# ElBaldo1/FastOptSolver

Measured on AMD Instinct MI355X. Metric: fista_iterations_per_second, higher is better.
Workload: dtype f32

## Files before the change

### fastoptsolver_amd/_core.py

```python
import ctypes as C
import collections
import math

import numpy as np
import torch

from . import _lib


def require_gpu():
    if not torch.cuda.is_available():
        raise _lib.FosError("fastoptsolver_amd needs a ROCm GPU (torch.cuda.is_available() is False); "
                            "there is no CPU fallback by design")


def stream_ptr():
    return C.c_void_p(torch.cuda.current_stream().cuda_stream)


def ptr(t):
    return C.c_void_p(t.data_ptr()) if t is not None else C.c_void_p(0)


def is_tensor(x):
# ... 416 lines not shown

    def plan(self):
        arr = (C.c_int32 * 8)()
        _lib.check(self.lib.fos_problem_plan(self.h, arr), "fos_problem_plan")
        keys = ("path", "threads", "chunks", "rows", "workgroups", "slabs", "nontemporal", "cus")
        plan = dict(zip(keys, list(arr)))
        flags = plan["nontemporal"]
        plan["nontemporal"] = flags & 1
        plan["resident"] = (flags >> 1) & 1
        plan["tall"] = (flags >> 2) & 1
        plan["colblock"] = (flags >> 3) & 1
        plan["cluster"] = (flags >> 4) & 1
        plan["interleave"] = (flags >> 5) & 1
        plan["fused_mfma"] = (flags >> 6) & 1
        plan["chip_resident"] = (flags >> 7) & 1
        return plan

    def replan(self, no_resident=False, no_tall=False, no_wide=False, no_colblock=False, cluster=None, interleave=None,
               fused_mfma=False, chip_resident=None):
        flags = ((_lib.PLAN_NO_RESIDENT if no_resident else 0) | (_lib.PLAN_NO_TALL if no_tall else 0) |
                 (_lib.PLAN_NO_WIDE if no_wide else 0) | (_lib.PLAN_NO_COLBLOCK if no_colblock else 0) |
                 (0 if cluster is None else (_lib.PLAN_CLUSTER if cluster else _lib.PLAN_NO_CLUSTER)) |
                 (0 if interleave is None else (_lib.PLAN_INTERLEAVE if interleave else _lib.PLAN_NO_INTERLEAVE)) |
                 (_lib.PLAN_FUSED_MFMA if fused_mfma else 0) |
                 (0 if chip_resident is None else (_lib.PLAN_CHIP_RESIDENT if chip_resident else _lib.PLAN_NO_CHIP_RESIDENT)))
        with self.ctx():
            _lib.check(self.lib.fos_problem_replan(self.h, flags), "fos_problem_replan")

    def set_comm(self, comm):
        _lib.check(self.lib.fos_problem_set_comm(self.h, comm.h if comm is not None else None), "fos_problem_set_comm")
        self.comm = comm

    def set_comm_cols(self, comm):
        with self.ctx():
            _lib.check(self.lib.fos_problem_set_comm_cols(self.h, comm.h), "fos_problem_set_comm_cols")
        self.comm = comm
        self.col_sharded = True

    def tune(self, threads, chunks, rows, workgroups=0):
        _lib.check(self.lib.fos_problem_tune(self.h, threads, chunks, rows, workgroups), "fos_problem_tune")
# ... 399 lines not shown
```

### fastoptsolver_amd/_lib.py

```python
import ctypes as C
import os

HERE = os.path.dirname(os.path.abspath(__file__))
LIB_PATH = os.path.join(HERE, "libfos_hip.so")

FOS_F32, FOS_BF16 = 0, 1
MODE_FISTA, MODE_DELTA, MODE_ISTA = 0, 1, 2
PROX_L1, PROX_ENET = 0, 1
LOSS_SQUARED, LOSS_LOGISTIC = 0, 1
LOSS_MULTINOMIAL = 2
STOP_NONE, STOP_STEP, STOP_RATIO, STOP_GRAD, STOP_LS_STALL = 0, 1, 2, 3, 4
ERR_UNSUPPORTED = -4
PLAN_NO_RESIDENT, PLAN_NO_TALL, PLAN_NO_WIDE, PLAN_NO_COLBLOCK, PLAN_CLUSTER, PLAN_INTERLEAVE, PLAN_NO_INTERLEAVE, PLAN_NO_CLUSTER, PLAN_FUSED_MFMA, PLAN_CHIP_RESIDENT, PLAN_NO_CHIP_RESIDENT = 1, 2, 4, 8, 16, 32, 64, 128, 256, 512, 1024


class FistaParams(C.Structure):
    _fields_ = [("tau", C.c_double), ("alpha1", C.c_double), ("alpha2", C.c_double), ("delta", C.c_double),
                ("restart_threshold", C.c_double), ("tol_step", C.c_double), ("tol_ratio", C.c_double),
                ("tol_grad", C.c_double), ("mode", C.c_int32), ("prox_kind", C.c_int32), ("adaptive_restart", C.c_int32),
                ("group", C.c_int32)]


class LineSearchState(C.Structure):
    _fields_ = [(k, C.c_double) for k in ("f0", "d0", "dtest", "width", "width1", "lo", "flo", "dlo", "hi", "fhi", "dhi",
                                           "smin", "smax")] + [(k, C.c_int32) for k in ("stage1", "brackt", "status", "reserved")]


class LbfgsResult(C.Structure):
# ... 161 lines not shown
```

### fastoptsolver_amd/csrc/fos_fista.hip

```cpp
#include "fos_internal.hpp"
#include "fused_step.hpp"
#include "chip_resident.hpp"
#include <cassert>

using namespace fosapi;

template <int NQ>
static int launch_fused(const fos::FusedArgs& a, int G, size_t lds, hipStream_t st) {
  auto kern = fos::fista_fused_kernel<NQ>;
  static std::atomic<uint64_t> done{0};
  int dev = 0;
  HIP_TRY(hipGetDevice(&dev));
  const uint64_t bit = 1ull << (dev & 63);
  if (!(done.load(std::memory_order_acquire) & bit)) {
    HIP_TRY(hipFuncSetAttribute(reinterpret_cast<const void*>(kern), hipFuncAttributeMaxDynamicSharedMemorySize, (int)lds));
    done.fetch_or(bit, std::memory_order_release);
  }
  hipLaunchKernelGGL(kern, dim3(G), dim3(fos::FZ_THREADS), lds, st, a);
  LAUNCH_CHECK();
  return FOS_OK;
}

template <int NC, bool CTRL>
static int launch_chip(const fos::ChipArgs& a, int G, size_t lds, hipStream_t st) {
// ... 402 lines not shown
  hipLaunchKernelGGL(fos::history_fold_kernel, dim3(iters), dim3(64), 0, p->stream, rr2_slots, nwg, part_slots, f->nupd,
                     hist);
  LAUNCH_CHECK();
  rc = finish_plain(f, part_slots + (iters - 1) * psz, iters >= 2 ? part_slots + (iters - 2) * psz : nullptr, f->nupd,
                    p->pass.rr_part, nwg);
  restart_plain(f);
  return rc;
}

int fos_fista_run(fos_fista* f, int iters) {
  if (!f || iters < 0) return fail(FOS_ERR_ARG, "fos_fista_run: bad argument");
  if (int rc_ = need_squared(f->p, "fos_fista_run")) return rc_;
  if (int rc_ = need_separable(f, "fos_fista_run")) return rc_;
  fos_problem* p = f->p;
  if (iters == 0) return FOS_OK;
  if (p->pass.resident) return run_resident(f, iters, nullptr, nullptr);
  {
    const bool chip_region = p->dtype == FOS_F32 && p->m >= 512 && iters >= 8 &&
                             (p->n <= 8 ? p->m <= 131072 : (p->n <= 16 && p->m <= 32768));
    if ((p->chip_mode == 1 || (p->chip_mode == 0 && chip_region)) && !p->comm && !f->precise && !f->prm.tau_from_state &&
        f->prm.tol_grad == 0.0) {
      const int rcc = fos_fista_run_chip(f, iters);
      if (rcc != FOS_ERR_UNSUPPORTED && rcc != FOS_ERR_STATE) return rcc;
    }
  }
  if (f->prm.tol_grad > 0.0 && !p->comm) {
    for (int it = 0; it < iters; ++it) {
      int rc;
      if ((rc = fos_fista_grad(f))) return rc;
      if ((rc = launch_grad_norm_stop(f))) return rc;
// ... 717 lines not shown
                       (int)p->cand.n_pad, f->x_cur, f->x_prev, f->scal, f->prm, t, eta, nv, p->cand.xp, p->ws.part, t_from_state);
  hipLaunchKernelGGL(fos::fold_partials_kernel, dim3(1), dim3(fos::FOLD_THREADS), 0, p->stream, p->ws.part, grid, fos::BT_W, p->cand.bt_out);
  LAUNCH_CHECK();
  if (p->col_sharded) {
    int rc = reduce_across(p, p->cand.bt_out, fos::BT_W, true);
    if (rc) return rc;
  }
  return launch_residual_batch(p, 0, p->cand.bt_out + 64, stopped);
}

static int run_device_driven(fos_fista* f, int iters, bool backtracking, double eta, double armijo_c, double grad_eps,
                             int32_t* ls_iters, double* tau_hist, double* x_hist, double* hist, double* rr_seen) {
  fos_problem* p = f->p;
  int rc = flush_pending(f);
  if (rc) return rc;
  if (backtracking) {
    if ((rc = ensure_batch_workspace(p))) return rc;
    if (!f->tau_on_device) {
      hipLaunchKernelGGL(fos::set_state_tau_kernel, dim3(1), dim3(1), 0, p->stream, f->scal, f->prm.tau);
      LAUNCH_CHECK();
      f->tau_on_device = true;
    }
  }
  hand_to_device(f);
  fos::FistaParams prm_dev = f->prm;
  prm_dev.tau_from_state = backtracking ? 1 : 0;
  const bool record = hist != nullptr;
  for (int it = 0; it < iters; ++it) {
    if (record && rr_seen != nullptr) {
      if ((rc = fos_fista_grad_dual(f))) return rc;
// ... 189 lines not shown
```

### fastoptsolver_amd/csrc/fos_internal.hpp

```cpp
#pragma once
#include <hip/hip_runtime.h>

#include <algorithm>
#include <atomic>
#include <cmath>
#include <cstdio>
#include <cstring>
#include <memory>
#include <string>
#include <chrono>
#include <vector>

#pragma GCC visibility push(default)
#include "../../include/fos.h"
#include "../../include/fos_feature_groups.h"
#pragma GCC visibility pop
#include "batch_trial.hpp"
#include "cluster_pass.hpp"
#include "comm.hpp"
#include "gemv_multi.hpp"
#include "gemv_pair.hpp"
#include "gemv_tall.hpp"
#include "gemv_wide.hpp"
#include "gram_batch.hpp"
// ... 169 lines not shown
  DevBuf<double> rdd;
  DevBuf<double> slabs;
  DevBuf<double> q_part;
  void reset() { *this = DdMultiPlan{}; }
};

struct CandPlan {
  bool planned = false;
  int64_t n_pad = 0;
  DevBuf<float> xp;
  DevBuf<double> q_part;
  DevBuf<double> bt_out;
  void reset() { *this = CandPlan{}; }
};

struct FeatureGroups {
  int32_t ngroups = 0;
  double l1_mix = 0.0;
  DevBuf<int32_t> start;
  DevBuf<float> weight;
  DevBuf<int32_t> of_coord;
  DevBuf<double> u;
  DevBuf<double> nrm2;
  void reset() { *this = FeatureGroups{}; }
};

struct Scratch {
  DevBuf<float> gbuf_own;
  DevBuf<float> ybuf;
  DevBuf<double> dscal;
// ... 22 lines not shown
  int loss = FOS_LOSS_SQUARED;
  int classes = 0;
  const float* row_weight = nullptr;
  const float* coord_factor = nullptr;
  const float* coord_lo = nullptr;
  const float* coord_hi = nullptr;
  hipStream_t stream = nullptr;
  int ncu = 256;
  bool col_sharded = false;
  unsigned plan_flags = 0;
  bool allow_resident = true;
  bool il = false;
  int dd_nwg_hint = 0;
  int cp_mode = 0;
  int chip_mode = 0;
  bool fused_on = false;
  unsigned cp_epoch = 1;
  PassPlan pass;
  DdPlan dd;
  MultiPlan multi;
  DdMultiPlan dm;
  CandPlan cand;
  FeatureGroups fg;
  Scratch ws;
  std::unique_ptr<LbfgsWork> lbfgs;
  std::unique_ptr<LbfgsMultiWork> lbfgs_multi;
  int profiling = 0;
  int64_t prof_seq = 0;
  bool prof_open = false;
  std::vector<hipEvent_t> ev_pool;
  size_t ev_used = 0;
  double prof_ms = 0.0;
  int64_t prof_launches = 0;
};

struct fos_fista {
  fos_problem* p = nullptr;
// ... 27 lines not shown
int grid_1d(int64_t n, int per_block, int cap);
void plan_fused(fos_problem* p, const MenuEntry* e, int nwg_hint);
void apply_plan(fos_problem* p, unsigned flags);
enum PlanInput : unsigned {
  IN_PLAN = 1,
  IN_TUNE = 2,
  IN_TUNE_DD = 4,
  IN_COMM = 8,
  IN_CLUSTER = 16,
};
int invalidate(fos_problem* p, unsigned changed);
int plan_multi_mfma(fos_problem* p);
int ensure_workspace(fos_problem* p);
int ensure_batch_workspace(fos_problem* p);
int ensure_dd(fos_problem* p);
int prof_drain(fos_problem* p);
int prof_mark(fos_problem* p, bool start);
int aligned_vec(fos_problem* p, const float* v, const float** out);
bool batch_supported(const fos_problem* p);
MultiLaunch find_multi(int64_t n, int nv, bool bblock = false);
int pack_candidates(fos_problem* p, const float* X, int nv);
int stage_b16(fos_problem* p, const float* B, int64_t ldb, int nv);
int launch_pass(fos_problem* p, const YSource& ys, const float* b, bool with_g, int* n_rr, bool dual = false,
                double* rr_to = nullptr);
int launch_slab_reduce(fos_problem* p, int n_rr, float* gbuf, double* rr_out, const int* stopped);
bool fold_held_block(const int32_t* held, int nv, fos::FoldHeld* out);
struct BatchLaunch {
  const void* A;
  const float* b;
  int use_b;
// ... 42 lines not shown
```

### fastoptsolver_amd/csrc/fos_plan.hip

```cpp
#include "fos_internal.hpp"
#include "softmax_link.hpp"

namespace fosapi {

thread_local std::string g_err;



template <typename T, int THREADS, int K, int R, int MINW, bool WITH_G, int NBUF, bool DUAL, bool DRAIN = false, bool CB = false,
          bool IL = false>
void fused_launch(const void* A, int64_t lda, const float* b, int64_t m, int n, YSource ys, int64_t rpw, float* slabs,
                  double* rr_part, double* rr2_part, int nwg, hipStream_t st) {
  hipLaunchKernelGGL((fos::gemv_pair_kernel<T, THREADS, K, R, true, MINW, WITH_G, NBUF, IL, DUAL, DRAIN, float, false, CB>), dim3(nwg),
                     dim3(THREADS), 0, st, reinterpret_cast<const T*>(A), lda, b, m, n, ys, rpw, slabs, rr_part,
                     rr2_part);
}


template <typename K>
int raise_dynamic_lds(K kernel, size_t bytes, std::atomic<uint64_t>& done) {
  int dev = 0;
  if (hipGetDevice(&dev) != hipSuccess) return FOS_ERR_HIP;
  const uint64_t bit = 1ull << (dev & 63);
  if (done.load(std::memory_order_acquire) & bit) return FOS_OK;
// ... 281 lines not shown
      if (rc) return rc;
    } else {
      for (int i = 0; i < 2; ++i) {
        hipEvent_t e;
        HIP_TRY(hipEventCreate(&e));
        p->ev_pool.push_back(e);
      }
    }
  }
  HIP_TRY(hipEventRecord(p->ev_pool[p->ev_used++], p->stream));
  return FOS_OK;
}

int launch_pass_inner(fos_problem* p, const YSource& ys, const float* b, bool with_g, int* n_rr, bool dual, double* rr_to);
int launch_pass(fos_problem* p, const YSource& ys, const float* b, bool with_g, int* n_rr, bool dual, double* rr_to) {
  int rc = prof_mark(p, true);
  if (rc) return rc;
  if ((rc = launch_pass_inner(p, ys, b, with_g, n_rr, dual, rr_to))) return rc;
  return prof_mark(p, false);
}


__global__ __launch_bounds__(256) void sumsq_partials_kernel(const float* __restrict__ v, int64_t m, double* __restrict__ part,
                                                            const int* stopped) {
  if (stopped != nullptr && *stopped != 0) return;
  __shared__ double ws[4];
  double acc = 0.0;
  for (int64_t i = (int64_t)blockIdx.x * 256 + threadIdx.x; i < m; i += (int64_t)gridDim.x * 256) acc += (double)v[i] * (double)v[i];
  acc = fos::wave_sum(acc);
  if ((threadIdx.x & 63) == 0) ws[threadIdx.x >> 6] = acc;
  __syncthreads();
  if (threadIdx.x == 0) part[blockIdx.x] = (ws[0] + ws[1]) + (ws[2] + ws[3]);
// ... 61 lines not shown
    return FOS_OK;
  }
  for (int cb = 0; cb < nblk; ++cb) {
    const int64_t c0 = cb * W;
    const int nb = (int)std::min<int64_t>(W, p->n - c0);
    YSource yz{p->pass.zeros, nullptr, nullptr, nullptr, ys.stopped};
    yz.slab_stride = p->n;
    p->pass.entry->with_g_cb(Ab + c0 * esz, p->lda, p->pass.rneg, p->m, nb, yz, p->pass.rows_per_wg, p->pass.slabs + c0, cb == 0 ? p->pass.rr_part : p->pass.rr2_part,
                        p->pass.rr2_part, p->pass.nwg, p->stream);
    LAUNCH_CHECK();
  }
  *n_rr = p->pass.nwg;
  return FOS_OK;
}

int launch_pass_inner(fos_problem* p, const YSource& ys, const float* b, bool with_g, int* n_rr, bool dual, double* rr_to) {
  if (p->pass.path == 0 && p->pass.colblock) return launch_pass_colblock(p, ys, b, with_g, n_rr);
  if (p->pass.path == 0) {
    FusedLaunch fn = dual ? p->pass.entry->dual : (with_g ? p->pass.entry->with_g : p->pass.entry->resid_only);
    if (p->il) {
      FusedLaunch fi = dual ? p->pass.entry->dual_il : (with_g ? p->pass.entry->with_g_il : p->pass.entry->resid_only_il);
      if (fi) fn = fi;
    }
    fn(p->A, p->lda, b, p->m, (int)p->n, ys, p->pass.rows_per_wg, p->pass.slabs, rr_to && !dual ? rr_to : p->pass.rr_part.get(),
       rr_to && dual ? rr_to : p->pass.rr2_part.get(), p->pass.nwg, p->stream);
    LAUNCH_CHECK();
    *n_rr = p->pass.nwg;
    return FOS_OK;
  }
  int rc = launch_residual_rows(p, ys, b, p->pass.resid_grid, p->pass.rr_part);
  if (rc) return rc;
  *n_rr = p->pass.resid_grid;
// ... 423 lines not shown
  const bool vec_ok = vec_layout(p);
  int64_t cb_width = 0;
  const MenuEntry* e = vec_ok ? default_entry(p->dtype, n) : nullptr;
  if ((n <= fos::TL_MAX_N || (n <= tlr_max_n(p->dtype) && vec_ok)) && !(flags & FOS_PLAN_NO_TALL))
    plan_tall(p, tall_entry(p->dtype, n, p->lda, p->A));
  else if (e) plan_fused(p, e, 0);
  else if (vec_ok && n <= fos::WD_MAX_N && !(flags & FOS_PLAN_NO_WIDE)) plan_fused(p, wide_entry(p->dtype), 0);
  else if (const MenuEntry* ce = (vec_ok && !(flags & FOS_PLAN_NO_COLBLOCK)) ? colblock_entry(p, &cb_width) : nullptr)
    plan_colblock(p, ce, cb_width);
  else plan_fallback(p);
}

int invalidate(fos_problem* p, unsigned changed) {
  if (changed & (IN_TUNE_DD | IN_CLUSTER)) HIP_TRY(hipStreamSynchronize(p->stream));
  if (changed & IN_PLAN) p->pass.reset();
  if (changed & IN_COMM) plan_resident(p);
  if (changed & (IN_PLAN | IN_TUNE | IN_TUNE_DD | IN_COMM)) p->dd.reset();
  if (changed & (IN_PLAN | IN_COMM | IN_CLUSTER)) p->multi.reset();
  return FOS_OK;
}

int plan_multi_mfma(fos_problem* p) {
  if (p->multi.planned) return FOS_OK;
  int rc;
  const bool is_bf16 = p->dtype == FOS_BF16;
  const int cs_need = (int)((p->n + fos::CP_W - 1) / fos::CP_W);
  const bool cluster_wins = (p->n == 4096 || p->n == 8192) && p->m * p->n >= (1ll << 29) && !p->comm;
  const bool want_cluster = p->cp_mode == 1 || (p->cp_mode == 0 && cluster_wins);
  if (want_cluster && !is_bf16 && p->ncu % 8 == 0) {
    const int cs = cs_need <= 2 ? 0 : cs_need <= 4 ? 4 : cs_need <= 8 ? 8 : cs_need <= 16 ? 16 : 0;
// ... 358 lines not shown
  hipEvent_t ev;
  HIP_TRY(hipEventCreateWithFlags(&ev, hipEventDisableTiming));
  hipError_t e = hipEventRecord(ev, p->stream);
  if (e == hipSuccess) e = hipStreamWaitEvent(ns, ev, 0);
  (void)hipEventDestroy(ev);
  if (e != hipSuccess) return fail(FOS_ERR_HIP, std::string("fos_problem_set_stream: ") + hipGetErrorString(e));
  p->stream = ns;
  return FOS_OK;
}

int fos_problem_replan(fos_problem* p, unsigned flags) {
  if (!p) return fail(FOS_ERR_ARG, "fos_problem_replan: null");
  if (p->col_sharded) return fail(FOS_ERR_UNSUPPORTED, "fos_problem_replan: a column-sharded problem keeps its two-phase plan");
  if (flags & ~(unsigned)(FOS_PLAN_NO_RESIDENT | FOS_PLAN_NO_TALL | FOS_PLAN_NO_WIDE | FOS_PLAN_NO_COLBLOCK | FOS_PLAN_CLUSTER |
                           FOS_PLAN_INTERLEAVE | FOS_PLAN_NO_INTERLEAVE | FOS_PLAN_NO_CLUSTER | FOS_PLAN_FUSED_MFMA |
                           FOS_PLAN_CHIP_RESIDENT | FOS_PLAN_NO_CHIP_RESIDENT))
    return fail(FOS_ERR_ARG, "fos_problem_replan: unknown flag");
  p->cp_mode = (flags & FOS_PLAN_CLUSTER) ? 1 : (flags & FOS_PLAN_NO_CLUSTER) ? 2 : 0;
  p->fused_on = (flags & FOS_PLAN_FUSED_MFMA) != 0;
  p->chip_mode = (flags & FOS_PLAN_CHIP_RESIDENT) ? 1 : (flags & FOS_PLAN_NO_CHIP_RESIDENT) ? 2 : 0;
  flags &= ~(unsigned)(FOS_PLAN_CLUSTER | FOS_PLAN_NO_CLUSTER | FOS_PLAN_FUSED_MFMA | FOS_PLAN_CHIP_RESIDENT |
                       FOS_PLAN_NO_CHIP_RESIDENT);
  int rc = invalidate(p, IN_PLAN);
  if (rc) return rc;
  apply_plan(p, flags);
  return ensure_workspace(p);
}

int fos_stream_read_probe(const void* buf, size_t bytes, int launches, void* stream, double* gbps_out, double* us_out) {
  if (!buf || bytes < 16 || (bytes & 15) || (reinterpret_cast<uintptr_t>(buf) & 15) || launches < 1 || !gbps_out)
    return fail(FOS_ERR_ARG, "fos_stream_read_probe: needs a 16-byte aligned buffer of a multiple of 16 bytes and launches >= 1");
  hipStream_t st = reinterpret_cast<hipStream_t>(stream);
  int dev = 0, ncu = 0;
  HIP_TRY(hipGetDevice(&dev));
  HIP_TRY(hipDeviceGetAttribute(&ncu, hipDeviceAttributeMultiprocessorCount, dev));
  const size_t n16 = bytes / 16;
  const int grid = (int)std::max<size_t>(1, std::min<size_t>((size_t)ncu, (n16 + 4095) / 4096));
// ... 51 lines not shown
  for (hipEvent_t e : p->ev_pool) (void)hipEventDestroy(e);
  delete p;
  return FOS_OK;
}

int fos_problem_plan(const fos_problem* p, int32_t plan[8]) {
  if (!p || !plan) return fail(FOS_ERR_ARG, "fos_problem_plan: null");
  plan[0] = p->pass.path;
  plan[1] = p->pass.entry ? p->pass.entry->threads : 256;
  plan[2] = p->pass.entry ? p->pass.entry->k : 0;
  plan[3] = p->pass.entry ? p->pass.entry->r : 0;
  plan[4] = p->pass.nwg;
  plan[5] = p->pass.nslabs;
  plan[6] = (p->pass.path == 0 ? 1 : 0) | (p->pass.resident ? 2 : 0) | (p->pass.tall ? 4 : 0) | (p->pass.colblock ? 8 : 0) | (p->multi.cp_cs ? 16 : 0) |
            ((p->il && p->pass.entry && p->pass.entry->with_g_il && p->pass.path == 0 && !p->pass.colblock && !p->pass.tall) ? 32 : 0) |
            (p->fused_on ? 64 : 0) | (p->chip_mode == 1 ? 128 : 0);
  plan[7] = p->ncu;
  return FOS_OK;
}

int fos_problem_tune(fos_problem* p, int threads, int chunks, int rows, int workgroups) {
  if (!p) return fail(FOS_ERR_ARG, "fos_problem_tune: null");
  if (p->pass.path == 0 && p->pass.tall && workgroups > 0) {
    p->pass.rows_per_wg = ((p->m + workgroups - 1) / workgroups + 3) / 4 * 4;
    p->pass.nwg = (int)((p->m + p->pass.rows_per_wg - 1) / p->pass.rows_per_wg);
    p->pass.nslabs = p->pass.nwg;
    if (int rc = invalidate(p, IN_TUNE)) return rc;
    return ensure_workspace(p);
  }
  if (p->pass.path != 0 || p->pass.tall || p->pass.colblock)
    return fail(FOS_ERR_UNSUPPORTED, "fos_problem_tune: only the streaming single-pass kernel has a geometry menu");
// ... 420 lines not shown
```

### include/fos.h

```cpp
#ifndef FOS_H_
#define FOS_H_

#include <stdint.h>

#ifdef __cplusplus
extern "C" {
#endif

#define FOS_ABI_VERSION 3

enum { FOS_OK = 0, FOS_ERR_ARG = -1, FOS_ERR_HIP = -2, FOS_ERR_STATE = -3, FOS_ERR_UNSUPPORTED = -4 };
enum { FOS_F32 = 0, FOS_BF16 = 1 };
enum { FOS_MODE_FISTA = 0, FOS_MODE_DELTA = 1, FOS_MODE_ISTA = 2 };
enum { FOS_PROX_L1 = 0, FOS_PROX_ENET = 1 };
enum { FOS_LOSS_SQUARED = 0, FOS_LOSS_LOGISTIC = 1, FOS_LOSS_MULTINOMIAL = 2 };
enum { FOS_STOP_NONE = 0, FOS_STOP_STEP = 1, FOS_STOP_RATIO = 2, FOS_STOP_GRAD = 3, FOS_STOP_LS_STALL = 4 };

enum { FOS_PLAN_NO_RESIDENT = 1, FOS_PLAN_NO_TALL = 2, FOS_PLAN_NO_WIDE = 4, FOS_PLAN_NO_COLBLOCK = 8,
       FOS_PLAN_CLUSTER = 16,
       FOS_PLAN_INTERLEAVE = 32,
       FOS_PLAN_NO_INTERLEAVE = 64,
       FOS_PLAN_NO_CLUSTER = 128,
       FOS_PLAN_FUSED_MFMA = 256,
       FOS_PLAN_CHIP_RESIDENT = 512,
       FOS_PLAN_NO_CHIP_RESIDENT = 1024  };

typedef struct fos_problem fos_problem;
typedef struct fos_comm fos_comm;
typedef struct fos_fista fos_fista;

typedef struct fos_fista_params {
  double tau;
  double alpha1;
  double alpha2;
  double delta;
  double restart_threshold;
  double tol_step;
  double tol_ratio;
  double tol_grad;
  int32_t mode;
// ... 169 lines not shown
```

Measured before the change: 104.9.

## Add exponent-window packed storage of A with sparse exception correction for GEMV pass

Adds a one-time packing step that stores each f32 entry of A in 28 bits (a shared 4-bit exponent window plus 24 bits of mantissa and sign), cutting the bytes the bandwidth-bound streaming pass reads. Entries whose exponent falls outside the window are replaced by placeholders and stored in CSR/CSC exception lists, which two small kernels use to correct the residual and the gradient so the result stays exact. By default packing turns on only for large f32 problems (at least 2 GiB, n above 8192) served by the single-pass streaming kernel with few exceptions. The costs are host-side sampling and sorting during setup, extra device memory, and two extra kernel launches per pass when exceptions exist.

Measured after the change: 112.8, median of 6. +7.6%, better.

```diff
diff --git a/fastoptsolver_amd/_core.py b/fastoptsolver_amd/_core.py
--- a/fastoptsolver_amd/_core.py
+++ b/fastoptsolver_amd/_core.py
@@ -454,16 +454,18 @@
         plan["interleave"] = (flags >> 5) & 1
         plan["fused_mfma"] = (flags >> 6) & 1
         plan["chip_resident"] = (flags >> 7) & 1
+        plan["packed"] = (flags >> 8) & 1
         return plan
 
     def replan(self, no_resident=False, no_tall=False, no_wide=False, no_colblock=False, cluster=None, interleave=None,
-               fused_mfma=False, chip_resident=None):
+               fused_mfma=False, chip_resident=None, pack=None):
         flags = ((_lib.PLAN_NO_RESIDENT if no_resident else 0) | (_lib.PLAN_NO_TALL if no_tall else 0) |
                  (_lib.PLAN_NO_WIDE if no_wide else 0) | (_lib.PLAN_NO_COLBLOCK if no_colblock else 0) |
                  (0 if cluster is None else (_lib.PLAN_CLUSTER if cluster else _lib.PLAN_NO_CLUSTER)) |
                  (0 if interleave is None else (_lib.PLAN_INTERLEAVE if interleave else _lib.PLAN_NO_INTERLEAVE)) |
                  (_lib.PLAN_FUSED_MFMA if fused_mfma else 0) |
-                 (0 if chip_resident is None else (_lib.PLAN_CHIP_RESIDENT if chip_resident else _lib.PLAN_NO_CHIP_RESIDENT)))
+                 (0 if chip_resident is None else (_lib.PLAN_CHIP_RESIDENT if chip_resident else _lib.PLAN_NO_CHIP_RESIDENT)) |
+                 (0 if pack is None else (_lib.PLAN_PACK if pack else _lib.PLAN_NO_PACK)))
         with self.ctx():
             _lib.check(self.lib.fos_problem_replan(self.h, flags), "fos_problem_replan")
 
diff --git a/fastoptsolver_amd/_lib.py b/fastoptsolver_amd/_lib.py
--- a/fastoptsolver_amd/_lib.py
+++ b/fastoptsolver_amd/_lib.py
@@ -11,7 +11,7 @@
 LOSS_MULTINOMIAL = 2
 STOP_NONE, STOP_STEP, STOP_RATIO, STOP_GRAD, STOP_LS_STALL = 0, 1, 2, 3, 4
 ERR_UNSUPPORTED = -4
-PLAN_NO_RESIDENT, PLAN_NO_TALL, PLAN_NO_WIDE, PLAN_NO_COLBLOCK, PLAN_CLUSTER, PLAN_INTERLEAVE, PLAN_NO_INTERLEAVE, PLAN_NO_CLUSTER, PLAN_FUSED_MFMA, PLAN_CHIP_RESIDENT, PLAN_NO_CHIP_RESIDENT = 1, 2, 4, 8, 16, 32, 64, 128, 256, 512, 1024
+PLAN_NO_RESIDENT, PLAN_NO_TALL, PLAN_NO_WIDE, PLAN_NO_COLBLOCK, PLAN_CLUSTER, PLAN_INTERLEAVE, PLAN_NO_INTERLEAVE, PLAN_NO_CLUSTER, PLAN_FUSED_MFMA, PLAN_CHIP_RESIDENT, PLAN_NO_CHIP_RESIDENT, PLAN_PACK, PLAN_NO_PACK = 1, 2, 4, 8, 16, 32, 64, 128, 256, 512, 1024, 2048, 4096
 
 
 class FistaParams(C.Structure):
diff --git a/fastoptsolver_amd/csrc/fos_fista.hip b/fastoptsolver_amd/csrc/fos_fista.hip
--- a/fastoptsolver_amd/csrc/fos_fista.hip
+++ b/fastoptsolver_amd/csrc/fos_fista.hip
@@ -440,6 +440,7 @@
   if (int rc_ = need_separable(f, "fos_fista_run")) return rc_;
   fos_problem* p = f->p;
   if (iters == 0) return FOS_OK;
+  if (int rc_ = ensure_packed(p)) return rc_;
   if (p->pass.resident) return run_resident(f, iters, nullptr, nullptr);
   {
     const bool chip_region = p->dtype == FOS_F32 && p->m >= 512 && iters >= 8 &&
@@ -1187,6 +1188,7 @@
   fos_problem* p = f->p;
   int rc = flush_pending(f);
   if (rc) return rc;
+  if ((rc = ensure_packed(p))) return rc;
   if (backtracking) {
     if ((rc = ensure_batch_workspace(p))) return rc;
     if (!f->tau_on_device) {
diff --git a/fastoptsolver_amd/csrc/fos_internal.hpp b/fastoptsolver_amd/csrc/fos_internal.hpp
--- a/fastoptsolver_amd/csrc/fos_internal.hpp
+++ b/fastoptsolver_amd/csrc/fos_internal.hpp
@@ -207,6 +207,18 @@
   void reset() { *this = CandPlan{}; }
 };
 
+struct PackPlan {
+  bool tried = false, active = false;
+  int threads = 0;
+  unsigned e0 = 0;
+  int64_t nnz = 0;
+  DevBuf<unsigned char> P;
+  DevBuf<int> csr_ptr, csr_col, csc_ptr, csc_row;
+  DevBuf<float> csr_tv, csr_pv, csc_tv, csc_pv;
+  DevBuf<float> bprime, r;
+  void reset() { *this = PackPlan{}; }
+};
+
 struct FeatureGroups {
   int32_t ngroups = 0;
   double l1_mix = 0.0;
@@ -259,6 +271,7 @@
   int dd_nwg_hint = 0;
   int cp_mode = 0;
   int chip_mode = 0;
+  int pack_mode = 0;
   bool fused_on = false;
   unsigned cp_epoch = 1;
   PassPlan pass;
@@ -266,6 +279,7 @@
   MultiPlan multi;
   DdMultiPlan dm;
   CandPlan cand;
+  PackPlan pk;
   FeatureGroups fg;
   Scratch ws;
   std::unique_ptr<LbfgsWork> lbfgs;
@@ -323,6 +337,7 @@
 int ensure_workspace(fos_problem* p);
 int ensure_batch_workspace(fos_problem* p);
 int ensure_dd(fos_problem* p);
+int ensure_packed(fos_problem* p);
 int prof_drain(fos_problem* p);
 int prof_mark(fos_problem* p, bool start);
 int aligned_vec(fos_problem* p, const float* v, const float** out);
diff --git a/fastoptsolver_amd/csrc/fos_plan.hip b/fastoptsolver_amd/csrc/fos_plan.hip
--- a/fastoptsolver_amd/csrc/fos_plan.hip
+++ b/fastoptsolver_amd/csrc/fos_plan.hip
@@ -1,5 +1,6 @@
 #include "fos_internal.hpp"
 #include "softmax_link.hpp"
+#include "gemv_packed.hpp"
 
 namespace fosapi {
 
@@ -319,8 +320,9 @@
 
 int launch_pass_inner(fos_problem* p, const YSource& ys, const float* b, bool with_g, int* n_rr, bool dual, double* rr_to);
 int launch_pass(fos_problem* p, const YSource& ys, const float* b, bool with_g, int* n_rr, bool dual, double* rr_to) {
-  int rc = prof_mark(p, true);
-  if (rc) return rc;
+  int rc;
+  if (p->pack_mode == 1 && !p->pk.tried && with_g && !dual && (rc = ensure_packed(p))) return rc;
+  if ((rc = prof_mark(p, true))) return rc;
   if ((rc = launch_pass_inner(p, ys, b, with_g, n_rr, dual, rr_to))) return rc;
   return prof_mark(p, false);
 }
@@ -412,8 +414,168 @@
   return FOS_OK;
 }
 
+constexpr int64_t PACK_MIN_BYTES = 2ll << 30;
+constexpr int64_t PACK_MIN_N = 8193;
+constexpr double PACK_MAX_EXCEPTIONS = 1e-3;
+
+bool vec_layout(const fos_problem* p);
+bool pack_served(const fos_problem* p) {
+  const PassPlan& w = p->pass;
+  return p->dtype == FOS_F32 && w.path == 0 && !w.tall && !w.colblock && !w.resident && !p->col_sharded && w.entry != nullptr &&
+         w.entry != wide_entry(FOS_F32) && p->n % fos::pk::CPT == 0 && p->n <= 16384 && p->m < (1ll << 31) - 1 && vec_layout(p);
+}
+
+unsigned pack_window(const int64_t (&hist)[256]) {
+  unsigned best = 2;
+  int64_t best_cnt = -1;
+  for (unsigned e0 = 2; e0 <= fos::pk::E0_MAX; e0 += 2) {
+    int64_t c = 0;
+    for (unsigned e = e0; e < e0 + 16; ++e) c += hist[e];
+    if (c > best_cnt) { best_cnt = c; best = e0; }
+  }
+  return best;
+}
+
+int ensure_packed(fos_problem* p) {
+  namespace pk = fos::pk;
+  PackPlan& k = p->pk;
+  if (k.tried) return FOS_OK;
+  k.tried = true;
+  const int64_t m = p->m, n = p->n;
+  if (p->pack_mode == 2 || !pack_served(p)) return FOS_OK;
+  if (p->pack_mode == 0 && (m * n * 4 < PACK_MIN_BYTES || n < PACK_MIN_N)) return FOS_OK;
+  const int threads = n <= 8192 ? 512 : 1024;
+  const size_t p_bytes = (size_t)m * (size_t)pk::row_bytes(threads);
+  HIP_TRY(hipStreamSynchronize(p->stream));
+  size_t free_b = 0, total_b = 0;
+  HIP_TRY(hipMemGetInfo(&free_b, &total_b));
+  const size_t need = p_bytes + (size_t)((double)m * n * PACK_MAX_EXCEPTIONS) * 32 + (size_t)m * 16 + p_bytes / 16 + ((size_t)256 << 20);
+  if (free_b < need) return FOS_OK;
+  const float* A = static_cast<const float*>(p->A);
+
+  unsigned e0;
+  {
+    const int64_t srows = std::min<int64_t>(m, std::max<int64_t>(1, (4ll << 20) / n)), stride = m / srows;
+    std::vector<float> sample((size_t)srows * n);
+    HIP_TRY(hipMemcpy2D(sample.data(), (size_t)n * 4, A, (size_t)stride * p->lda * 4, (size_t)n * 4, (size_t)srows, hipMemcpyDeviceToHost));
+    int64_t hist[256] = {0};
+    for (float v : sample) {
+      unsigned u;
+      std::memcpy(&u, &v, 4);
+      ++hist[(u >> 23) & 0xffu];
+    }
+    e0 = pack_window(hist);
+  }
+  const int grid = (int)std::max<int64_t>(1, std::min<int64_t>((m * threads + 255) / 256, (int64_t)p->ncu * 32));
+  auto refuse = [&]() { k.reset(); k.tried = true; return FOS_OK; };
+
+  DevBuf<int> row_cnt;
+  DevBuf<unsigned> flags;
+  if (row_cnt.reserve((size_t)m) || flags.reserve(1)) return refuse();
+  HIP_TRY(hipMemsetAsync(row_cnt, 0, (size_t)m * sizeof(int), p->stream));
+  HIP_TRY(hipMemsetAsync(flags, 0, sizeof(unsigned), p->stream));
+  hipLaunchKernelGGL(pk::pack_rows_kernel<true>, dim3(grid), dim3(256), 0, p->stream, A, p->lda, m, (int)n, threads, e0,
+                     (unsigned char*)nullptr, row_cnt.get(), flags.get(), (const int*)nullptr, (int*)nullptr, (float*)nullptr,
+                     (float*)nullptr);
+  LAUNCH_CHECK();
+  std::vector<int> ptr((size_t)m + 1);
+  unsigned hflags = 0;
+  HIP_TRY(hipMemcpyAsync(ptr.data() + 1, row_cnt, (size_t)m * sizeof(int), hipMemcpyDeviceToHost, p->stream));
+  HIP_TRY(hipMemcpyAsync(&hflags, flags, sizeof(unsigned), hipMemcpyDeviceToHost, p->stream));
+  HIP_TRY(hipStreamSynchronize(p->stream));
+  if (hflags) return refuse();
+  int64_t nnz = 0;
+  ptr[0] = 0;
+  for (int64_t i = 1; i <= m; ++i) {
+    nnz += ptr[i];
+    if (nnz > (1ll << 30)) return refuse();
+    ptr[i] = (int)nnz;
+  }
+  if ((double)nnz > PACK_MAX_EXCEPTIONS * (double)m * (double)n) return refuse();
+
+  const size_t cap = (size_t)std::max<int64_t>(nnz, 1);
+  if (k.P.reserve(p_bytes) || k.csr_ptr.reserve((size_t)m + 1) || k.csr_col.reserve(cap) || k.csr_tv.reserve(cap) ||
+      k.csr_pv.reserve(cap) || k.csc_ptr.reserve((size_t)n + 1) || k.csc_row.reserve(cap) || k.csc_tv.reserve(cap) ||
+      k.csc_pv.reserve(cap) || k.bprime.reserve((size_t)m) || k.r.reserve((size_t)m))
+    return refuse();
+  HIP_TRY(hipMemcpyAsync(k.csr_ptr, ptr.data(), ((size_t)m + 1) * sizeof(int), hipMemcpyHostToDevice, p->stream));
+  HIP_TRY(hipMemsetAsync(row_cnt, 0, (size_t)m * sizeof(int), p->stream));
+  hipLaunchKernelGGL(pk::pack_rows_kernel<false>, dim3(grid), dim3(256), 0, p->stream, A, p->lda, m, (int)n, threads, e0, k.P.get(),
+                     row_cnt.get(), flags.get(), (const int*)k.csr_ptr.get(), k.csr_col.get(), k.csr_tv.get(), k.csr_pv.get());
+  LAUNCH_CHECK();
+  HIP_TRY(hipStreamSynchronize(p->stream));
+
+  if (nnz > 0) {
+    std::vector<int> col((size_t)nnz), row((size_t)nnz), perm;
+    std::vector<float> tv((size_t)nnz), pv((size_t)nnz), tv2((size_t)nnz), pv2((size_t)nnz);
+    std::vector<int> col2((size_t)nnz), cptr((size_t)n + 1, 0);
+    HIP_TRY(hipMemcpy(col.data(), k.csr_col, (size_t)nnz * sizeof(int), hipMemcpyDeviceToHost));
+    HIP_TRY(hipMemcpy(tv.data(), k.csr_tv, (size_t)nnz * sizeof(float), hipMemcpyDeviceToHost));
+    HIP_TRY(hipMemcpy(pv.data(), k.csr_pv, (size_t)nnz * sizeof(float), hipMemcpyDeviceToHost));
+    for (int64_t i = 0; i < m; ++i) {
+      const int lo = ptr[i], hi = ptr[i + 1];
+      if (lo == hi) continue;
+      perm.resize((size_t)(hi - lo));
+      for (int q = lo; q < hi; ++q) perm[(size_t)(q - lo)] = q;
+      std::sort(perm.begin(), perm.end(), [&](int a, int b) { return col[(size_t)a] < col[(size_t)b]; });
+      for (int q = lo; q < hi; ++q) {
+        const size_t src = (size_t)perm[(size_t)(q - lo)];
+        col2[(size_t)q] = col[src]; tv2[(size_t)q] = tv[src]; pv2[(size_t)q] = pv[src];
+        ++cptr[(size_t)col[src] + 1];
+      }
+    }
+    for (int64_t j = 0; j < n; ++j) cptr[(size_t)j + 1] += cptr[(size_t)j];
+    std::vector<int> fill(cptr.begin(), cptr.end() - 1);
+    for (int64_t i = 0; i < m; ++i)
+      for (int q = ptr[i]; q < ptr[i + 1]; ++q) {
+        const size_t dst = (size_t)fill[(size_t)col2[(size_t)q]]++;
+        row[dst] = (int)i; tv[dst] = tv2[(size_t)q]; pv[dst] = pv2[(size_t)q];
+      }
+    HIP_TRY(hipMemcpy(k.csr_col, col2.data(), (size_t)nnz * sizeof(int), hipMemcpyHostToDevice));
+    HIP_TRY(hipMemcpy(k.csr_tv, tv2.data(), (size_t)nnz * sizeof(float), hipMemcpyHostToDevice));
+    HIP_TRY(hipMemcpy(k.csr_pv, pv2.data(), (size_t)nnz * sizeof(float), hipMemcpyHostToDevice));
+    HIP_TRY(hipMemcpy(k.csc_ptr, cptr.data(), ((size_t)n + 1) * sizeof(int), hipMemcpyHostToDevice));
+    HIP_TRY(hipMemcpy(k.csc_row, row.data(), (size_t)nnz * sizeof(int), hipMemcpyHostToDevice));
+    HIP_TRY(hipMemcpy(k.csc_tv, tv.data(), (size_t)nnz * sizeof(float), hipMemcpyHostToDevice));
+    HIP_TRY(hipMemcpy(k.csc_pv, pv.data(), (size_t)nnz * sizeof(float), hipMemcpyHostToDevice));
+  }
+  k.threads = threads;
+  k.e0 = e0;
+  k.nnz = nnz;
+  k.active = true;
+  return FOS_OK;
+}
+
+int launch_pass_packed(fos_problem* p, const YSource& ys, const float* b, int* n_rr, double* rr_to) {
+  namespace pk = fos::pk;
+  PackPlan& k = p->pk;
+  const float* bp = b;
+  if (k.nnz > 0) {
+    hipLaunchKernelGGL(pk::pk_bprime_kernel, dim3((unsigned)((p->m + 255) / 256)), dim3(256), 0, p->stream, (const int*)k.csr_ptr.get(),
+                       (const int*)k.csr_col.get(), (const float*)k.csr_tv.get(), (const float*)k.csr_pv.get(), b, p->m, ys,
+                       k.bprime.get());
+    LAUNCH_CHECK();
+    bp = k.bprime;
+  }
+  auto kern = k.threads == 1024 ? (p->il ? pk::gemv_packed_kernel<1024, true> : pk::gemv_packed_kernel<1024, false>)
+                                : (p->il ? pk::gemv_packed_kernel<512, true> : pk::gemv_packed_kernel<512, false>);
+  hipLaunchKernelGGL(kern, dim3(p->pass.nwg), dim3(k.threads), 0, p->stream, (const unsigned char*)k.P.get(), bp, p->m, (int)p->n, ys,
+                     (k.e0 >> 1) * 0x01010101u, p->pass.rows_per_wg, p->pass.slabs.get(), k.r.get(),
+                     rr_to ? rr_to : p->pass.rr_part.get());
+  LAUNCH_CHECK();
+  if (k.nnz > 0) {
+    hipLaunchKernelGGL(pk::pk_dtr_kernel, dim3((unsigned)((p->n + 3) / 4)), dim3(256), 0, p->stream, (const int*)k.csc_ptr.get(),
+                       (const int*)k.csc_row.get(), (const float*)k.csc_tv.get(), (const float*)k.csc_pv.get(), (const float*)k.r.get(),
+                       (int)p->n, ys.stopped, p->pass.slabs.get());
+    LAUNCH_CHECK();
+  }
+  *n_rr = p->pass.nwg;
+  return FOS_OK;
+}
+
 int launch_pass_inner(fos_problem* p, const YSource& ys, const float* b, bool with_g, int* n_rr, bool dual, double* rr_to) {
   if (p->pass.path == 0 && p->pass.colblock) return launch_pass_colblock(p, ys, b, with_g, n_rr);
+  if (p->pk.active && with_g && !dual) return launch_pass_packed(p, ys, b, n_rr, rr_to);
   if (p->pass.path == 0) {
     FusedLaunch fn = dual ? p->pass.entry->dual : (with_g ? p->pass.entry->with_g : p->pass.entry->resid_only);
     if (p->il) {
@@ -867,6 +1029,7 @@
 int invalidate(fos_problem* p, unsigned changed) {
   if (changed & (IN_TUNE_DD | IN_CLUSTER)) HIP_TRY(hipStreamSynchronize(p->stream));
   if (changed & IN_PLAN) p->pass.reset();
+  if (changed & (IN_PLAN | IN_TUNE | IN_COMM)) p->pk.reset();
   if (changed & IN_COMM) plan_resident(p);
   if (changed & (IN_PLAN | IN_TUNE | IN_TUNE_DD | IN_COMM)) p->dd.reset();
   if (changed & (IN_PLAN | IN_COMM | IN_CLUSTER)) p->multi.reset();
@@ -1255,13 +1418,14 @@
   if (p->col_sharded) return fail(FOS_ERR_UNSUPPORTED, "fos_problem_replan: a column-sharded problem keeps its two-phase plan");
   if (flags & ~(unsigned)(FOS_PLAN_NO_RESIDENT | FOS_PLAN_NO_TALL | FOS_PLAN_NO_WIDE | FOS_PLAN_NO_COLBLOCK | FOS_PLAN_CLUSTER |
                            FOS_PLAN_INTERLEAVE | FOS_PLAN_NO_INTERLEAVE | FOS_PLAN_NO_CLUSTER | FOS_PLAN_FUSED_MFMA |
-                           FOS_PLAN_CHIP_RESIDENT | FOS_PLAN_NO_CHIP_RESIDENT))
+                           FOS_PLAN_CHIP_RESIDENT | FOS_PLAN_NO_CHIP_RESIDENT | FOS_PLAN_PACK | FOS_PLAN_NO_PACK))
     return fail(FOS_ERR_ARG, "fos_problem_replan: unknown flag");
   p->cp_mode = (flags & FOS_PLAN_CLUSTER) ? 1 : (flags & FOS_PLAN_NO_CLUSTER) ? 2 : 0;
   p->fused_on = (flags & FOS_PLAN_FUSED_MFMA) != 0;
   p->chip_mode = (flags & FOS_PLAN_CHIP_RESIDENT) ? 1 : (flags & FOS_PLAN_NO_CHIP_RESIDENT) ? 2 : 0;
+  p->pack_mode = (flags & FOS_PLAN_NO_PACK) ? 2 : (flags & FOS_PLAN_PACK) ? 1 : 0;
   flags &= ~(unsigned)(FOS_PLAN_CLUSTER | FOS_PLAN_NO_CLUSTER | FOS_PLAN_FUSED_MFMA | FOS_PLAN_CHIP_RESIDENT |
-                       FOS_PLAN_NO_CHIP_RESIDENT);
+                       FOS_PLAN_NO_CHIP_RESIDENT | FOS_PLAN_PACK | FOS_PLAN_NO_PACK);
   int rc = invalidate(p, IN_PLAN);
   if (rc) return rc;
   apply_plan(p, flags);
@@ -1343,7 +1507,7 @@
   plan[5] = p->pass.nslabs;
   plan[6] = (p->pass.path == 0 ? 1 : 0) | (p->pass.resident ? 2 : 0) | (p->pass.tall ? 4 : 0) | (p->pass.colblock ? 8 : 0) | (p->multi.cp_cs ? 16 : 0) |
             ((p->il && p->pass.entry && p->pass.entry->with_g_il && p->pass.path == 0 && !p->pass.colblock && !p->pass.tall) ? 32 : 0) |
-            (p->fused_on ? 64 : 0) | (p->chip_mode == 1 ? 128 : 0);
+            (p->fused_on ? 64 : 0) | (p->chip_mode == 1 ? 128 : 0) | (p->pk.active ? 256 : 0);
   plan[7] = p->ncu;
   return FOS_OK;
 }
diff --git a/fastoptsolver_amd/csrc/gemv_packed.hpp b/fastoptsolver_amd/csrc/gemv_packed.hpp
--- /dev/null
+++ b/fastoptsolver_amd/csrc/gemv_packed.hpp
@@ -0,0 +1,263 @@
+#pragma once
+#include "gemv_pair.hpp"
+
+namespace fos {
+namespace pk {
+
+typedef float f32x2 __attribute__((ext_vector_type(2)));
+typedef unsigned u32x2 __attribute__((ext_vector_type(2)));
+
+constexpr int CPT = 16;
+constexpr int BYTES_PER_THREAD = 56;
+constexpr unsigned E0_MAX = 238;
+
+__host__ __device__ inline int64_t row_bytes(int threads) { return (int64_t)threads * BYTES_PER_THREAD; }
+
+__host__ __device__ inline bool in_window(unsigned bits, unsigned e0) {
+  const unsigned ex = (bits >> 23) & 0xffu;
+  return ex >= e0 && ex <= e0 + 15u;
+}
+__host__ __device__ inline unsigned placeholder(unsigned bits, unsigned e0) {
+  const unsigned ex = (bits >> 23) & 0xffu;
+  return (bits & 0x807fffffu) | ((ex < e0 ? e0 : e0 + 15u) << 23);
+}
+__host__ __device__ inline unsigned nibble_of(unsigned bits, unsigned e0) {
+  return ((bits >> 31) << 3) | ((((bits >> 23) & 0xffu) - e0) >> 1);
+}
+__host__ __device__ inline void pack16(const unsigned (&bits)[CPT], unsigned e0, unsigned (&pl)[3][4], unsigned (&nb)[2]) {
+  nb[0] = nb[1] = 0;
+#pragma unroll
+  for (int g = 0; g < 4; ++g) {
+    const unsigned d = bits[4 * g + 3];
+    pl[0][g] = (bits[4 * g] & 0xffffffu) | ((d & 0xffu) << 24);
+    pl[1][g] = (bits[4 * g + 1] & 0xffffffu) | (((d >> 8) & 0xffu) << 24);
+    pl[2][g] = (bits[4 * g + 2] & 0xffffffu) | (((d >> 16) & 0xffu) << 24);
+#pragma unroll
+    for (int k = 0; k < 4; ++k) nb[g >> 1] |= nibble_of(bits[4 * g + k], e0) << (8u * k + 4u * (g & 1));
+  }
+}
+
+__device__ inline unsigned top_bytes(unsigned w, unsigned e0h4) {
+  unsigned t = w & 0x0F0F0F0Fu;
+  t += 0x78787878u;
+  t &= 0x87878787u;
+  return t + e0h4;
+}
+__device__ inline void decode_group(unsigned p0, unsigned p1, unsigned p2, unsigned top, float (&f)[4]) {
+  f[0] = __uint_as_float(__builtin_amdgcn_perm(top, p0, 0x04020100u));
+  f[1] = __uint_as_float(__builtin_amdgcn_perm(top, p1, 0x05020100u));
+  f[2] = __uint_as_float(__builtin_amdgcn_perm(top, p2, 0x06020100u));
+  const unsigned d01 = __builtin_amdgcn_perm(p1, p0, 0x0c0c0703u);
+  const unsigned d012 = __builtin_amdgcn_perm(p2, d01, 0x0c070100u);
+  f[3] = __uint_as_float(__builtin_amdgcn_perm(top, d012, 0x07020100u));
+}
+__device__ inline u32x2 load8nt(const void* p) { return __builtin_nontemporal_load(reinterpret_cast<const u32x2*>(p)); }
+
+template <int THREADS, bool IL>
+__global__ __launch_bounds__(THREADS, THREADS / 256) void gemv_packed_kernel(
+    const unsigned char* __restrict__ P, const float* __restrict__ b, int64_t m, int n, YSource ys, unsigned e0h4,
+    int64_t rows_per_wg, float* __restrict__ slabs, float* __restrict__ r_out, double* __restrict__ rr_part) {
+  constexpr int NW = THREADS / 64;
+  constexpr int NBUF = 2;
+  static_assert(NW >= 8 && NW <= 64, "one partial per lane in the cross-wave sum");
+  __shared__ float red[2][NW];
+
+  if (ys.stopped != nullptr && *ys.stopped != 0) return;
+  if (ys.t_stamp != nullptr && blockIdx.x == 0 && threadIdx.x == 0) *ys.t_stamp = wall_clock64();
+
+  const int tid = threadIdx.x, lane = tid & 63, wave = tid >> 6;
+  const int64_t row_lo = IL ? 0 : (int64_t)blockIdx.x * rows_per_wg;
+  int64_t row_hi = IL ? m : row_lo + rows_per_wg;
+  if (row_hi > m) row_hi = m;
+
+  const int col = tid * CPT;
+  const bool live = col < n;
+  f32x2 yv[CPT / 2], gv[CPT / 2];
+#pragma unroll
+  for (int e = 0; e < CPT / 2; ++e) { yv[e] = f32x2{0.f, 0.f}; gv[e] = f32x2{0.f, 0.f}; }
+  if (live) {
+    const double beta = source_beta(ys);
+#pragma unroll
+    for (int q = 0; q < CPT / 4; ++q) {
+      if (ys.y != nullptr) {
+        const f32x4 t = *reinterpret_cast<const f32x4*>(ys.y + col + 4 * q);
+        yv[2 * q] = f32x2{t.x, t.y}; yv[2 * q + 1] = f32x2{t.z, t.w};
+      } else {
+        yv[2 * q] = f32x2{(float)source_y(ys, col + 4 * q, beta), (float)source_y(ys, col + 4 * q + 1, beta)};
+        yv[2 * q + 1] = f32x2{(float)source_y(ys, col + 4 * q + 2, beta), (float)source_y(ys, col + 4 * q + 3, beta)};
+      }
+    }
+  }
+
+  const int64_t nrows = row_hi - row_lo;
+  const int64_t group = IL ? gridDim.x : 1;
+  const int64_t first = IL ? (int64_t)blockIdx.x : 0;
+  const int64_t nsteps = nrows > first ? (nrows - first + group - 1) / group : 0;
+  const int64_t rbytes = row_bytes(THREADS);
+  const unsigned voff16 = (unsigned)tid * 16u, voff8 = (unsigned)THREADS * 48u + (unsigned)tid * 8u;
+  double rr = 0.0;
+
+  u32x4 tile[NBUF][3];
+  u32x2 nib[NBUF];
+  float bval[NBUF];
+  const float* b_src = b != nullptr ? b : reinterpret_cast<const float*>(P);
+  auto issue = [&](int buf, int64_t step) {
+    int64_t row = row_lo + first + step * group;
+    if (row >= row_hi) row = row_hi - 1;
+    bval[buf] = b_src[b != nullptr ? row : 0];
+    const unsigned char* rp = P + row * rbytes;
+#pragma unroll
+    for (int c = 0; c < 3; ++c) tile[buf][c] = load16<true>(rp + voff16 + (unsigned)c * THREADS * 16u);
+    nib[buf] = load8nt(rp + voff8);
+  };
+  auto consume = [&](int buf, int64_t step) {
+    f32x2 a[CPT / 2];
+#pragma unroll
+    for (int g = 0; g < 4; ++g) {
+      const unsigned w = (g >> 1) ? nib[buf].y : nib[buf].x;
+      const unsigned top = top_bytes((g & 1) ? (w >> 4) : w, e0h4);
+      float f[4];
+      decode_group(tile[buf][0][g], tile[buf][1][g], tile[buf][2][g], top, f);
+      a[2 * g] = f32x2{f[0], f[1]}; a[2 * g + 1] = f32x2{f[2], f[3]};
+    }
+    f32x2 acc0 = f32x2{0.f, 0.f}, acc1 = f32x2{0.f, 0.f};
+#pragma unroll
+    for (int e = 0; e < CPT / 2; e += 2) {
+      acc0 = __builtin_elementwise_fma(a[e], yv[e], acc0);
+      acc1 = __builtin_elementwise_fma(a[e + 1], yv[e + 1], acc1);
+    }
+    acc0 += acc1;
+    const float part = wave_sum(acc0.x + acc0.y);
+    const int pb = (int)(step & 1);
+    if (lane == 0) red[pb][wave] = part;
+    __syncthreads();
+    float s = wave_sum(lane < NW ? red[pb][lane] : 0.f);
+    const int64_t row = row_lo + first + step * group;
+    const float bi = b != nullptr ? bval[buf] : 0.f;
+    if (row < row_hi) {
+      s -= bi;
+      rr += (double)s * (double)s;
+      if (tid == 0) r_out[row] = s;
+    } else {
+      s = 0.f;
+    }
+    const f32x2 s2 = f32x2{s, s};
+#pragma unroll
+    for (int e = 0; e < CPT / 2; ++e) gv[e] = __builtin_elementwise_fma(a[e], s2, gv[e]);
+  };
+
+  if (nsteps > 0) {
+    issue(0, 0);
+    int64_t s = 0;
+    for (; s + NBUF <= nsteps; s += NBUF) {
+#pragma unroll
+      for (int u = 0; u < NBUF; ++u) {
+        issue((u + NBUF - 1) % NBUF, s + u + NBUF - 1);
+        asm volatile("s_waitcnt vmcnt(0)" ::: "memory");
+        __builtin_amdgcn_sched_barrier(0);
+        consume(u, s + u);
+        __builtin_amdgcn_sched_barrier(0);
+      }
+    }
+    if (s < nsteps) consume(0, s);
+  }
+
+  if (live) {
+    float* slab = slabs + (int64_t)blockIdx.x * n + col;
+#pragma unroll
+    for (int q = 0; q < CPT / 4; ++q)
+      *reinterpret_cast<f32x4*>(slab + 4 * q) = f32x4{gv[2 * q].x, gv[2 * q].y, gv[2 * q + 1].x, gv[2 * q + 1].y};
+  }
+  if (tid == 0) rr_part[blockIdx.x] = rr;
+}
+
+template <bool COUNT>
+__global__ __launch_bounds__(256) void pack_rows_kernel(const float* __restrict__ A, int64_t lda, int64_t m, int n, int threads,
+                                                        unsigned e0, unsigned char* __restrict__ P, int* __restrict__ row_cnt,
+                                                        unsigned* __restrict__ flags, const int* __restrict__ csr_ptr,
+                                                        int* __restrict__ csr_col, float* __restrict__ csr_tv,
+                                                        float* __restrict__ csr_pv) {
+  const int64_t total = m * threads;
+  for (int64_t i = (int64_t)blockIdx.x * blockDim.x + threadIdx.x; i < total; i += (int64_t)gridDim.x * blockDim.x) {
+    const int64_t row = i / threads;
+    const int t = (int)(i % threads);
+    unsigned pl[3][4] = {{0, 0, 0, 0}, {0, 0, 0, 0}, {0, 0, 0, 0}};
+    unsigned nb[2] = {0, 0};
+    if (t * CPT < n) {
+      const float* ap = A + row * lda + (int64_t)t * CPT;
+      unsigned bits[CPT];
+#pragma unroll
+      for (int q = 0; q < CPT / 4; ++q) {
+        const u32x4 v = *reinterpret_cast<const u32x4*>(ap + 4 * q);
+        bits[4 * q] = v.x; bits[4 * q + 1] = v.y; bits[4 * q + 2] = v.z; bits[4 * q + 3] = v.w;
+      }
+      int nex = 0;
+      bool bad = false;
+#pragma unroll
+      for (int e = 0; e < CPT; ++e) {
+        if (in_window(bits[e], e0)) continue;
+        ++nex;
+        bad |= ((bits[e] >> 23) & 0xffu) == 0xffu;
+        if constexpr (!COUNT) {
+          const unsigned ph = placeholder(bits[e], e0);
+          const int slot = csr_ptr[row] + atomicAdd(&row_cnt[row], 1);
+          csr_col[slot] = t * CPT + e;
+          csr_tv[slot] = __uint_as_float(bits[e]);
+          csr_pv[slot] = __uint_as_float(ph);
+          bits[e] = ph;
+        }
+      }
+      if constexpr (COUNT) {
+        if (nex) atomicAdd(&row_cnt[row], nex);
+        if (bad) atomicOr(flags, 1u);
+      } else {
+        pack16(bits, e0, pl, nb);
+      }
+    }
+    if constexpr (!COUNT) {
+      unsigned char* rp = P + row * row_bytes(threads);
+#pragma unroll
+      for (int c = 0; c < 3; ++c)
+        *reinterpret_cast<u32x4*>(rp + (int64_t)c * threads * 16 + (int64_t)t * 16) = u32x4{pl[c][0], pl[c][1], pl[c][2], pl[c][3]};
+      *reinterpret_cast<u32x2*>(rp + (int64_t)threads * 48 + (int64_t)t * 8) = u32x2{nb[0], nb[1]};
+    }
+  }
+}
+
+static __global__ __launch_bounds__(256) void pk_bprime_kernel(const int* __restrict__ csr_ptr, const int* __restrict__ csr_col,
+                                                              const float* __restrict__ csr_tv, const float* __restrict__ csr_pv,
+                                                              const float* __restrict__ b, int64_t m, YSource ys,
+                                                              float* __restrict__ bprime) {
+  if (ys.stopped != nullptr && *ys.stopped != 0) return;
+  const int64_t i = (int64_t)blockIdx.x * 256 + threadIdx.x;
+  if (i >= m) return;
+  const double beta = source_beta(ys);
+  double acc = 0.0;
+  for (int k = csr_ptr[i]; k < csr_ptr[i + 1]; ++k) {
+    const double y = (double)(float)source_y(ys, csr_col[k], beta);
+    acc = fma((double)csr_tv[k], y, acc);
+    acc = fma(-(double)csr_pv[k], y, acc);
+  }
+  bprime[i] = (float)((b != nullptr ? (double)b[i] : 0.0) - acc);
+}
+static __global__ __launch_bounds__(256) void pk_dtr_kernel(const int* __restrict__ csc_ptr, const int* __restrict__ csc_row,
+                                                           const float* __restrict__ csc_tv, const float* __restrict__ csc_pv,
+                                                           const float* __restrict__ r, int n, const int* stopped,
+                                                           float* __restrict__ slab0) {
+  if (stopped != nullptr && *stopped != 0) return;
+  const int j = blockIdx.x * 4 + (threadIdx.x >> 6), lane = threadIdx.x & 63;
+  if (j >= n) return;
+  const int lo = csc_ptr[j], hi = csc_ptr[j + 1];
+  if (lo == hi) return;
+  double acc = 0.0;
+  for (int k = lo + lane; k < hi; k += 64) {
+    const double ri = (double)r[csc_row[k]];
+    acc = fma((double)csc_tv[k], ri, acc);
+    acc = fma(-(double)csc_pv[k], ri, acc);
+  }
+  acc = wave_sum(acc);
+  if (lane == 0) slab0[j] = (float)((double)slab0[j] + acc);
+}
+
+}
+}
diff --git a/include/fos.h b/include/fos.h
--- a/include/fos.h
+++ b/include/fos.h
@@ -23,7 +23,9 @@
        FOS_PLAN_NO_CLUSTER = 128,
        FOS_PLAN_FUSED_MFMA = 256,
        FOS_PLAN_CHIP_RESIDENT = 512,
-       FOS_PLAN_NO_CHIP_RESIDENT = 1024  };
+       FOS_PLAN_NO_CHIP_RESIDENT = 1024,
+       FOS_PLAN_PACK = 2048,
+       FOS_PLAN_NO_PACK = 4096       };
 
 typedef struct fos_problem fos_problem;
 typedef struct fos_comm fos_comm;
```
